# jackroos/VL-BERT

Measured on AMD Instinct MI355X. Metric: samples/sec VL-BERT-base pretrain (seq 64+36 regions) at 1/2/4/8 MI355X, higher is better.
Workload: dtype bf16; 1 GPU; VL-BERT-base 12-layer pretrain step (fwd+bwd+clip+AdamW), 64 text + 36 regions, precomputed 2048-d region features, dropout on; global_batch=256, per_gpu_batch=256, per_gpu_caption_samples=256, per_gpu_text_only_samples=0, module=ResNetVLBERTForPretraining, seq_len=101, parallelism=dp1, hipgraph=False, arch=gfx950:sramecc+:xnack-, cus=256, forced_exchange=False, ranks=1

## Files before the change

### vl-bert_amd/csrc/gemm_p8.hip

```cpp
#include <math.h>
#include <stdlib.h>
#include <string.h>

#include <type_traits>

#include "gemm_params.h"

#ifndef VLB_P8_LN_SB
#define VLB_P8_LN_SB 2
#endif
#ifndef VLB_P8_SIDE_DEPTH
#define VLB_P8_SIDE_DEPTH 1
#endif
#ifndef VLB_P8_WDRAIN
#define VLB_P8_WDRAIN 1
#endif

namespace {

template <int OFF>
__device__ __forceinline__ void p8_lds_read(bf16x8& dst, uint32_t vaddr) {
  asm volatile("ds_read_b128 %0, %1 offset:%2" : "=v"(dst) : "v"(vaddr), "n"(OFF));
}

template <int OFF>
__device__ __forceinline__ void p8_lds_write_f4(uint32_t vaddr, const f32x4& v) {
  asm volatile("ds_write_b128 %0, %1 offset:%2" : : "v"(vaddr), "v"(v), "n"(OFF) : "memory");
}

template <int OFF>
__device__ __forceinline__ void p8_lds_read_f4(f32x4& dst, uint32_t vaddr) {
  asm volatile("ds_read_b128 %0, %1 offset:%2" : "=v"(dst) : "v"(vaddr), "n"(OFF));
}

template <int OFF>
__device__ __forceinline__ void p8_stage_read(f32x4& x0, f32x4& x1, uint32_t a0, uint32_t a1) {
  asm volatile("ds_read_b128 %0, %2 offset:%4\n\tds_read_b128 %1, %3 offset:%4\n\ts_waitcnt lgkmcnt(0)"
               : "=&v"(x0), "=&v"(x1) : "v"(a0), "v"(a1), "n"(OFF) : "memory");
}

template <int I, int N, typename F>
__device__ __forceinline__ void p8_static_for(F&& f) {
  if constexpr (I < N) {
    f(std::integral_constant<int, I>{});
    p8_static_for<I + 1, N>(f);
  }
}

__device__ __forceinline__ void p8_barrier() {
  asm volatile("" ::: "memory");
  __builtin_amdgcn_s_barrier();
  asm volatile("" ::: "memory");
}

template <int EPI>
__device__ __forceinline__ void p8_epilogue8(const GemmParams& p, float (&v)[8], const float (&b8)[8], int m, int n, uint32_t seed,
                                             const uint4& side, const float2 ms = make_float2(0.f, 0.f), const float* g8 = nullptr,
                                             const float* be8 = nullptr) {
#pragma unroll
  for (int e = 0; e < 8; ++e) v[e] += b8[e];
  if (EPI == 1) {
    float d[8];
#pragma unroll
    for (int e = 0; e < 8; e += 2) {
      vlb_f2 g2, d2;
      gelu_both2((vlb_f2){v[e], v[e + 1]}, g2, d2);
      v[e] = g2.x; v[e + 1] = g2.y;
      d[e] = d2.x; d[e + 1] = d2.y;
    }
    if (p.pre) {
      const uint4 dv = make_uint4(pack2bf(d[0], d[1]), pack2bf(d[2], d[3]), pack2bf(d[4], d[5]), pack2bf(d[6], d[7]));
      vlb_store_nt((uint4*)(p.pre + (long)m * p.ldpre + n), dv);
    }
  } else if (EPI == 2) {
    v[0] *= bflo(side.x); v[1] *= bfhi(side.x); v[2] *= bflo(side.y); v[3] *= bfhi(side.y);
    v[4] *= bflo(side.z); v[5] *= bfhi(side.z); v[6] *= bflo(side.w); v[7] *= bfhi(side.w);
  } else if (EPI == 5) {
#pragma unroll
    for (int e = 0; e < 8; ++e) v[e] = fmaxf(v[e], 0.f);
  }
  if (EPI == 3 || EPI == 6) {
    const uint32_t idx = (uint32_t)m * (uint32_t)p.N + (uint32_t)n;
    if ((idx & 1u) == 0) {
#pragma unroll
      for (int q = 0; q < 4; ++q) {
        const uint32_t h = vlb_rng_pair(seed, p.tag, (idx >> 1) + q);
        v[2 * q] = ((h & 0xffffu) >= p.drop_thr) ? v[2 * q] * p.drop_scale : 0.f;
        v[2 * q + 1] = ((h >> 16) >= p.drop_thr) ? v[2 * q + 1] * p.drop_scale : 0.f;
      }
    } else {
#pragma unroll
      for (int e = 0; e < 8; ++e) v[e] = vlb_keep(seed, p.tag, idx + e, p.drop_thr) ? v[e] * p.drop_scale : 0.f;
    }
  }
  if (EPI == 3 || EPI == 4 || EPI == 8) {
    v[0] += bflo(side.x); v[1] += bfhi(side.x); v[2] += bflo(side.y); v[3] += bfhi(side.y);
    v[4] += bflo(side.z); v[5] += bfhi(side.z); v[6] += bflo(side.w); v[7] += bfhi(side.w);
  }
  if (EPI == 8) {
#pragma unroll
    for (int e = 0; e < 8; ++e) v[e] = fmaxf(v[e], 0.f);
  }
  if (EPI == 10) {
    const float a[8] = {bflo(side.x), bfhi(side.x), bflo(side.y), bfhi(side.y), bflo(side.z), bfhi(side.z), bflo(side.w), bfhi(side.w)};
#pragma unroll
    for (int e = 0; e < 8; ++e) v[e] = a[e] > 0.f ? v[e] : 0.f;
  }
  if (EPI == 6 || EPI == 7) {
    const float z[8] = {hlo(side.x), hhi(side.x), hlo(side.y), hhi(side.y), hlo(side.z), hhi(side.z), hlo(side.w), hhi(side.w)};
#pragma unroll
    for (int e = 0; e < 8; ++e) v[e] += fmaf((z[e] - ms.x) * ms.y, g8[e], be8[e]);
  }
}

template <int EPI>
__device__ __forceinline__ float p8_epilogue1(const GemmParams& p, float v, int m, int n, uint32_t seed) {
  if (p.bias) v += p.bias[n];
  if (EPI == 1) {
    float g, d;
    gelu_both(v, g, d);
    if (p.pre) p.pre[(long)m * p.ldpre + n] = f2bf(d);
    v = g;
  } else if (EPI == 2) {
    v *= bf2f(p.aux[(long)m * p.ldaux + n]);
  } else if (EPI == 5) {
    v = fmaxf(v, 0.f);
  }
  if (EPI == 3 || EPI == 6) v = vlb_keep(seed, p.tag, (uint32_t)m * (uint32_t)p.N + (uint32_t)n, p.drop_thr) ? v * p.drop_scale : 0.f;
  if (EPI == 3 || EPI == 4 || EPI == 8) v += bf2f(p.res[(long)m * p.ldres + n]);
  if (EPI == 8) v = fmaxf(v, 0.f);
  if (EPI == 10) v = bf2f(p.aux[(long)m * p.ldaux + n]) > 0.f ? v : 0.f;
  if (EPI == 6 || EPI == 7)
    v += fmaf((h2f(p.res[(long)m * p.ldres + n]) - p.res_stats[2 * (long)m]) * p.res_stats[2 * (long)m + 1], p.res_gamma[n], p.res_beta[n]);
  return v;
}

template <int FMH, int EPI, int KF>
__device__ __forceinline__ void p8_drain(const GemmParams& p, f32x4 (&acc)[2 * FMH][4], uint32_t slab, int m0, int n0, int wm, int wn,
                                         int lane, int tid, uint32_t seed) {
  constexpr int AH = 32 * FMH, NF = 2 * FMH;
  constexpr bool ALT = (KF == 0);
  constexpr bool LNRES = (EPI == 6 || EPI == 7);
  constexpr int FPR = ALT ? 1 : KF;
  constexpr int ROUNDS = ALT ? 2 * NF : (NF + FPR - 1) / FPR;
  constexpr int PASSES = ALT ? 1 : 2 * FPR;
  constexpr bool SIDE = (EPI == 2 || EPI == 3 || EPI == 4 || EPI == 6 || EPI == 7 || EPI == 8 || EPI == 10);
  constexpr bool PRE_NEXT = SIDE && (PASSES <= 2);
  constexpr int SB = PRE_NEXT ? PASSES : (FMH == 5 ? (LNRES ? VLB_P8_LN_SB : 4) : PASSES);
  asm volatile("" : "+v"(tid));
  lane = tid & 63;
  const int frow = lane & 15;
  const int wrow = (ALT ? 0 : wm * 16) + frow;
  uint32_t wr[4];
#pragma unroll
  for (int cj = 0; cj < 4; ++cj) {
#if VLB_P8_WDRAIN
    const int c = wn * 16 + (cj >> 1) * 8 + (cj & 1) * 4 + (lane >> 4);
#else
    const int c = (cj >> 1) * 32 + wn * 8 + (cj & 1) * 4 + (lane >> 4);
#endif
    wr[cj] = slab + (uint32_t)(wrow * 1024 + ((c ^ (frow & 7)) << 4));
  }
  const int q = tid & 31, rho = tid >> 5;
  const uint32_t rd0 = slab + (uint32_t)(rho * 1024 + (((2 * q) ^ (rho & 7)) << 4));
  const uint32_t rd1 = slab + (uint32_t)(rho * 1024 + (((2 * q + 1) ^ (rho & 7)) << 4));
  const int n = n0 + q * 8;
  const bool full8 = n + 8 <= p.N;
  bf16_t* const C = (bf16_t*)p.C;
  float b8[8] = {0.f, 0.f, 0.f, 0.f, 0.f, 0.f, 0.f, 0.f};
  if (p.bias && full8) {
    const float4 b0 = *(const float4*)(p.bias + n), b1 = *(const float4*)(p.bias + n + 4);
    b8[0] = b0.x; b8[1] = b0.y; b8[2] = b0.z; b8[3] = b0.w; b8[4] = b1.x; b8[5] = b1.y; b8[6] = b1.z; b8[7] = b1.w;
  }
  constexpr bool HOIST_GB = LNRES;
  float g8[8], be8[8];
  if constexpr (LNRES) {
#pragma unroll
    for (int e = 0; e < 8; ++e) g8[e] = be8[e] = 0.f;
    if (HOIST_GB && full8) {
      const float4 a0 = *(const float4*)(p.res_gamma + n), a1 = *(const float4*)(p.res_gamma + n + 4);
      const float4 c0 = *(const float4*)(p.res_beta + n), c1 = *(const float4*)(p.res_beta + n + 4);
      g8[0] = a0.x; g8[1] = a0.y; g8[2] = a0.z; g8[3] = a0.w; g8[4] = a1.x; g8[5] = a1.y; g8[6] = a1.z; g8[7] = a1.w;
      be8[0] = c0.x; be8[1] = c0.y; be8[2] = c0.z; be8[3] = c0.w; be8[4] = c1.x; be8[5] = c1.y; be8[6] = c1.z; be8[7] = c1.w;
    }
  }
  const bool f16out = p.c_f16 != 0;
  auto row_of = [&](int r, int pp) {
    const int f = ALT ? 0 : (pp >> 1), g = ALT ? (r & 1) : (pp & 1);
    const int R = ALT ? (r >> 1) : (r * FPR + f);
    const int ha = R / FMH, i = R - ha * FMH;
    return m0 + ha * AH + g * FMH * 16 + i * 16 + rho;
  };
  auto frag_valid = [&](int r, int pp) { return ALT ? true : (r * FPR + (pp >> 1) < NF); };
  auto load_side = [&](int r, int pp) {
    uint4 sd = make_uint4(0, 0, 0, 0);
    if constexpr (SIDE) {
      const int m = row_of(r, pp);
      if (frag_valid(r, pp) && m < p.M && full8) {
        if (EPI == 2 || EPI == 10) sd = vlb_load_nt((const uint4*)(p.aux + (long)m * p.ldaux + n));
        else sd = *(const uint4*)(p.res + (long)m * p.ldres + n);
      }
    }
    return sd;
  };
  auto load_ms = [&](int r, int pp) {
    float2 ms = make_float2(0.f, 0.f);
    if constexpr (LNRES) {
      const int m = min(max(row_of(r, pp), 0), p.M - 1);
      ms = *(const float2*)(p.res_stats + 2 * (long)m);
    }
    return ms;
  };
  uint4 side[2][SB];
  float2 mss[2][SB];
  if constexpr (PRE_NEXT) {
#pragma unroll
    for (int pp = 0; pp < PASSES; ++pp) {
      side[0][pp] = load_side(0, pp);
      mss[0][pp] = load_ms(0, pp);
    }
  }
  p8_static_for<0, ROUNDS>([&](auto r_c) {
    constexpr int r = decltype(r_c)::value;
    if constexpr (SIDE && !PRE_NEXT) {
#pragma unroll
      for (int pp = 0; pp < SB; ++pp) {
        side[0][pp] = load_side(r, pp);
        mss[0][pp] = load_ms(r, pp);
      }
    }
    if (!ALT || wm == (r & 1)) {
      p8_static_for<0, FPR>([&](auto f_c) {
        constexpr int f = decltype(f_c)::value;
        constexpr int R = ALT ? (r >> 1) : (r * FPR + f);
        if constexpr (R < NF) {
          const uint32_t o = (uint32_t)(f * 32 * 1024);
          p8_lds_write_f4<0>(wr[0] + o, acc[R][0]);
          p8_lds_write_f4<0>(wr[1] + o, acc[R][1]);
          p8_lds_write_f4<0>(wr[2] + o, acc[R][2]);
          p8_lds_write_f4<0>(wr[3] + o, acc[R][3]);
        }
      });
    }
    asm volatile("s_waitcnt lgkmcnt(0)" ::: "memory");
    p8_barrier();
    if constexpr (PRE_NEXT) {
      if (r + 1 < ROUNDS) {
#pragma unroll
        for (int pp = 0; pp < PASSES; ++pp) {
          side[(r + 1) & 1][pp] = load_side(r + 1, pp);
          mss[(r + 1) & 1][pp] = load_ms(r + 1, pp);
        }
      }
    }
#pragma unroll
    for (int pp = 0; pp < PASSES; ++pp) {
      if constexpr (SIDE && !PRE_NEXT) {
        if (pp > 0 && pp % SB == 0) {
#pragma unroll
          for (int k = 0; k < SB; ++k) {
            side[0][k] = load_side(r, pp + k);
            mss[0][k] = load_ms(r, pp + k);
          }
        }
      }
      if (!frag_valid(r, pp)) continue;
      const int m = row_of(r, pp);
      f32x4 x0, x1;
      p8_stage_read<0>(x0, x1, rd0 + (uint32_t)(pp * 16 * 1024), rd1 + (uint32_t)(pp * 16 * 1024));
      if (m < p.M && n < p.N) {
        float v[8] = {x0[0], x0[1], x0[2], x0[3], x1[0], x1[1], x1[2], x1[3]};
        if (full8) {
          const uint4 sd = SIDE ? (PRE_NEXT ? side[r & 1][pp] : side[0][pp % SB]) : make_uint4(0, 0, 0, 0);
          if constexpr (LNRES) {
            const float2 ms = PRE_NEXT ? mss[r & 1][pp] : mss[0][pp % SB];
            if constexpr (!HOIST_GB) {
              const float4 a0 = *(const float4*)(p.res_gamma + n), a1 = *(const float4*)(p.res_gamma + n + 4);
              const float4 c0 = *(const float4*)(p.res_beta + n), c1 = *(const float4*)(p.res_beta + n + 4);
              g8[0] = a0.x; g8[1] = a0.y; g8[2] = a0.z; g8[3] = a0.w; g8[4] = a1.x; g8[5] = a1.y; g8[6] = a1.z; g8[7] = a1.w;
              be8[0] = c0.x; be8[1] = c0.y; be8[2] = c0.z; be8[3] = c0.w; be8[4] = c1.x; be8[5] = c1.y; be8[6] = c1.z; be8[7] = c1.w;
            }
            p8_epilogue8<EPI>(p, v, b8, m, n, seed, sd, ms, g8, be8);
          } else {
            p8_epilogue8<EPI>(p, v, b8, m, n, seed, sd);
          }
          const uint4 o4 = make_uint4(pack2o(v[0], v[1], f16out), pack2o(v[2], v[3], f16out), pack2o(v[4], v[5], f16out), pack2o(v[6], v[7], f16out));
          if (p.ablate != 2) *(uint4*)(C + (long)m * p.ldc + n) = o4;
          else if (o4.x == 0x12345678u && o4.y == 0x9abcdef0u) C[0] = 1;
        } else {
          for (int e = 0; e < 8 && n + e < p.N; ++e) {
            const float o = p8_epilogue1<EPI>(p, v[e], m, n + e, seed);
            C[(long)m * p.ldc + n + e] = f16out ? f2h(o) : f2bf(o);
          }
        }
      }
    }
    if (r + 1 < ROUNDS) p8_barrier();
  });
  asm volatile("" ::"v"(b8[0]), "v"(b8[4]));
}

template <int FMH, int EPI, bool EDGE>
__device__ __forceinline__ void p8_drain_w(const GemmParams& p, f32x4 (&acc)[2 * FMH][4], uint32_t slab, int m0, int n0, int wm, int wn,
                                           int tid, uint32_t seed) {
  constexpr int AH = 32 * FMH, NF = 2 * FMH, NU = 2 * NF;
  constexpr bool LNRES = (EPI == 6 || EPI == 7);
  constexpr bool SIDE = (EPI == 2 || EPI == 3 || EPI == 4 || EPI == 6 || EPI == 7 || EPI == 8 || EPI == 10);
  asm volatile("" : "+v"(tid));
  const int lane = tid & 63, frow = lane & 15;
  const uint32_t mine = slab + (uint32_t)((tid >> 6) * 2048);
  uint32_t wr[4];
#pragma unroll
  for (int j = 0; j < 4; ++j) wr[j] = mine + (uint32_t)((frow & 7) * 256 + (((j * 4 + (lane >> 4)) ^ (frow & 7)) << 4));
  const bool upper = (frow >> 3) != 0;
  const int rr = lane >> 3, cq = lane & 7;
  const uint32_t rd0 = mine + (uint32_t)(rr * 256 + (((2 * cq) ^ rr) << 4));
  const uint32_t rd1 = mine + (uint32_t)(rr * 256 + (((2 * cq + 1) ^ rr) << 4));
  const bool f16out = p.c_f16 != 0;
  const int n = n0 + wn * 64 + cq * 8;
  const bool full8 = EDGE ? (n + 8 <= p.N) : true;
  const int mw = m0 + wm * FMH * 16 + rr;
  auto uoff = [](int u) { return ((u >> 1) / FMH) * AH + ((u >> 1) % FMH) * 16 + (u & 1) * 8; };
  bf16_t* const Cl = (bf16_t*)p.C + (long)mw * p.ldc + n;
  const bf16_t* const Sl = !SIDE ? nullptr : ((EPI == 2 || EPI == 10) ? p.aux + (long)mw * p.ldaux + n : p.res + (long)mw * p.ldres + n);
  const long lds_ = (EPI == 2 || EPI == 10) ? p.ldaux : p.ldres;
  const float* const Ml = LNRES ? p.res_stats + 2 * (long)mw : nullptr;
  float b8[8] = {0.f, 0.f, 0.f, 0.f, 0.f, 0.f, 0.f, 0.f}, g8[8], be8[8];
  auto consts = [&]() {
    if (p.bias && full8) {
      const float4 b0 = *(const float4*)(p.bias + n), b1 = *(const float4*)(p.bias + n + 4);
      b8[0] = b0.x; b8[1] = b0.y; b8[2] = b0.z; b8[3] = b0.w; b8[4] = b1.x; b8[5] = b1.y; b8[6] = b1.z; b8[7] = b1.w;
    }
    if constexpr (LNRES) {
#pragma unroll
      for (int e = 0; e < 8; ++e) g8[e] = be8[e] = 0.f;
      if (full8) {
        const float4 a0 = *(const float4*)(p.res_gamma + n), a1 = *(const float4*)(p.res_gamma + n + 4);
        const float4 c0 = *(const float4*)(p.res_beta + n), c1 = *(const float4*)(p.res_beta + n + 4);
        g8[0] = a0.x; g8[1] = a0.y; g8[2] = a0.z; g8[3] = a0.w; g8[4] = a1.x; g8[5] = a1.y; g8[6] = a1.z; g8[7] = a1.w;
        be8[0] = c0.x; be8[1] = c0.y; be8[2] = c0.z; be8[3] = c0.w; be8[4] = c1.x; be8[5] = c1.y; be8[6] = c1.z; be8[7] = c1.w;
      }
    }
  };
  auto load_side = [&](int u, uint4& sd, float2& ms) {
    if constexpr (SIDE) {
      if (!EDGE || (mw + uoff(u) < p.M && full8)) {
        const uint4* src = (const uint4*)(Sl + uoff(u) * lds_);
        if (EPI == 2 || EPI == 10) sd = vlb_load_nt(src);
        else sd = *src;
        if constexpr (LNRES) ms = *(const float2*)(Ml + 2 * uoff(u));
      }
    }
  };
  auto put = [&](auto u_c) {
    constexpr int u = decltype(u_c)::value, R = u >> 1, hf = u & 1;
    if (upper == (hf != 0)) {
      p8_lds_write_f4<0>(wr[0], acc[R][0]);
      p8_lds_write_f4<0>(wr[1], acc[R][1]);
      p8_lds_write_f4<0>(wr[2], acc[R][2]);
      p8_lds_write_f4<0>(wr[3], acc[R][3]);
    }
  };
  auto finish = [&](int u, const f32x4& x0, const f32x4& x1, const uint4& sd, const float2& ms) {
    const int m = mw + uoff(u);
    if (!EDGE || (m < p.M && n < p.N)) {
      float v[8] = {x0[0], x0[1], x0[2], x0[3], x1[0], x1[1], x1[2], x1[3]};
      if (full8) {
        if constexpr (LNRES) p8_epilogue8<EPI>(p, v, b8, m, n, seed, sd, ms, g8, be8);
        else p8_epilogue8<EPI>(p, v, b8, m, n, seed, sd);
        uint4 o4;
        if (f16out) {
          asm volatile("" ::: "memory");
          o4 = make_uint4(pack2h(v[0], v[1]), pack2h(v[2], v[3]), pack2h(v[4], v[5]), pack2h(v[6], v[7]));
        } else {
          o4 = make_uint4(pack2bf(v[0], v[1]), pack2bf(v[2], v[3]), pack2bf(v[4], v[5]), pack2bf(v[6], v[7]));
        }
        *(uint4*)(Cl + (p.ablate != 2 ? uoff(u) * (long)p.ldc : 0L)) = o4;
      } else {
        for (int e = 0; e < 8 && n + e < p.N; ++e) {
          const float o = p8_epilogue1<EPI>(p, v[e], m, n + e, seed);
          Cl[uoff(u) * (long)p.ldc + e] = f16out ? f2h(o) : f2bf(o);
        }
      }
    }
  };
  constexpr int DEPTH = (EPI == 2 || EPI == 10) ? VLB_P8_SIDE_DEPTH : 1, RING = DEPTH + 1;
  uint4 side[RING];
  float2 mst[RING];
#pragma unroll
  for (int d = 0; d < RING; ++d) {
    side[d] = make_uint4(0, 0, 0, 0);
    mst[d] = make_float2(0.f, 0.f);
  }
  consts();
  p8_static_for<0, (DEPTH < NU ? DEPTH : NU)>([&](auto d_c) {
    constexpr int d = decltype(d_c)::value;
    load_side(d, side[d % RING], mst[d % RING]);
  });
  put(std::integral_constant<int, 0>{});
  p8_static_for<0, NU>([&](auto u_c) {
    constexpr int u = decltype(u_c)::value;
    f32x4 x0, x1;
    p8_stage_read<0>(x0, x1, rd0, rd1);
    if constexpr (u + DEPTH < NU) load_side(u + DEPTH, side[(u + DEPTH) % RING], mst[(u + DEPTH) % RING]);
    if constexpr (u + 1 < NU) put(std::integral_constant<int, u + 1>{});
    finish(u, x0, x1, side[u % RING], mst[u % RING]);
  });
  asm volatile("" ::"v"(b8[0]), "v"(b8[4]));
}

template <int FMH, int EPI, bool KEEPB>
__global__ __launch_bounds__(512, 2) void gemm_nt_p8_kernel(const GemmParams p) {
  constexpr int AH = 32 * FMH;
  constexpr int BM = 2 * AH, BN = 256;
  constexpr int AHB = AH * 128, BHB = 128 * 128;
  constexpr int OFF_A0 = 0, OFF_A1 = AHB, OFF_B0 = 2 * AHB, OFF_B1 = 2 * AHB + BHB;
  constexpr int BUF = 2 * AHB + 2 * BHB;
  constexpr int STG = 2 * BUF;
  constexpr int SR = (163840 - STG) / 1024 >= 32 ? 32 : (163840 - STG) / 1024;
  constexpr int NLA = (AH * 8 + 511) / 512;
  constexpr int VM_AHEAD = (AH * 8) / 512 + 2;
  static_assert(SR == 32 || SR == 16, "staging slab");
  extern __shared__ __attribute__((aligned(16))) char smem[];

  const int tid = threadIdx.x, lane = tid & 63;
  const int wave = __builtin_amdgcn_readfirstlane(tid >> 6);
  const int wm = wave >> 2, wn = wave & 3;
  const int nt = p.ntm * p.ntn;
  const int nk = p.K >> 6;
  if ((int)blockIdx.x >= nt) return;
  unsigned long long* const stamps = (unsigned long long*)(EPI == 1 ? (void*)p.aux : (void*)p.pre);
  const bool stamp = (p.ablate == 4) && stamps;
  unsigned long long t_main = 0, t_epi = 0, t_mark = 0;
  if (stamp && tid == 0) {
    unsigned long long* t = stamps + 8 * blockIdx.x;
    t[0] = __builtin_readcyclecounter();
    t[1] = __builtin_amdgcn_s_memrealtime();
  }

  auto tile_of = [&](int w, int& m0, int& n0) {
    int tile_m, tile_n;
    vlb_tile_of(vlb_xcd_order(w, nt), p.ntm, p.ntn, p.tile_group, tile_m, tile_n);
    m0 = tile_m * BM;
    n0 = tile_n * BN;
  };

  const __amdgpu_buffer_rsrc_t rsA = __builtin_amdgcn_make_buffer_rsrc((void*)p.A, 0, 0x7FFFFFFF, 0x00020000);
  const __amdgpu_buffer_rsrc_t rsB = __builtin_amdgcn_make_buffer_rsrc((void*)p.B, 0, 0x7FFFFFFF, 0x00020000);
  const int ldaB = (int)p.lda * 2, ldbB = (int)p.ldb * 2;
  const int kcb = (((tid & 7) ^ ((tid >> 4) & 7)) << 4);
  const int rowA = (tid >> 3) * ldaB + kcb, maxA = (p.M - 1) * ldaB + kcb;
#if VLB_P8_WDRAIN
  const int rowB = ((tid >> 8) * 64 + ((tid >> 3) & 31)) * ldbB + kcb, maxB = (p.N - 1) * ldbB + kcb;
#else
  const int rowB = (tid >> 3) * ldbB + kcb, maxB = (p.N - 1) * ldbB + kcb;
#endif
  int w_p = blockIdx.x, kt_p = 0, pm0 = 0, pn0 = 0;
  auto setup = [&](int w) { tile_of(w, pm0, pn0); };
  auto stage = [&](auto which_c, auto buf_c) {
    constexpr int WHICH = decltype(which_c)::value, B_ = decltype(buf_c)::value;
    const int koff = kt_p * 128;
    if constexpr (WHICH < 2) {
      char* dst = smem + B_ * BUF + (WHICH == 0 ? OFF_A0 : OFF_A1);
#pragma unroll
      for (int it = 0; it < NLA; ++it) {
        if (it * 512 + 511 < AH * 8 || wave < (AH * 8 - it * 512) / 64) {
          const int vo = min((pm0 + WHICH * AH + it * 64) * ldaB + rowA, maxA);
          __builtin_amdgcn_raw_ptr_buffer_load_lds(rsA, LDS_PTR(dst + (it * 512 + wave * 64) * 16), 16, vo, koff, 0, 0);
        }
      }
    } else {
      char* dst = smem + B_ * BUF + (WHICH == 2 ? OFF_B0 : OFF_B1);
#pragma unroll
      for (int it = 0; it < 2; ++it) {
#if VLB_P8_WDRAIN
        const int vo = min((pn0 + (WHICH - 2) * 32 + it * 128) * ldbB + rowB, maxB);
#else
        const int vo = min((pn0 + (WHICH - 2) * 128 + it * 64) * ldbB + rowB, maxB);
#endif
        __builtin_amdgcn_raw_ptr_buffer_load_lds(rsB, LDS_PTR(dst + (it * 512 + wave * 64) * 16), 16, vo, koff, 0, 0);
      }
    }
  };
  auto advance = [&]() {
    if (++kt_p == nk) {
      if (w_p + (int)gridDim.x < nt) {
        kt_p = 0;
        w_p += gridDim.x;
        setup(w_p);
      } else {
        kt_p = nk - 1;
      }
    }
  };
  constexpr int ORD1 = KEEPB ? 2 : 3, ORD2 = KEEPB ? 3 : 1, ORD3 = KEEPB ? 1 : 2;
  using I0 = std::integral_constant<int, 0>;
  using I1 = std::integral_constant<int, 1>;
  using W0 = std::integral_constant<int, 0>;
  using W1 = std::integral_constant<int, ORD1>;
  using W2 = std::integral_constant<int, ORD2>;
  using W3 = std::integral_constant<int, ORD3>;

  f32x4 acc[2 * FMH][4];
  bf16x8 af[FMH][2], bfr[2][2], bkeep[2][2];
  const int frow = lane & 15;
  const uint32_t c0 = (uint32_t)((((lane >> 4) ^ (frow >> 1)) << 4));
  const uint32_t lds0 = (uint32_t)(uintptr_t)LDS_PTR(smem);
  const uint32_t a_rd = lds0 + (uint32_t)((wm * FMH * 16 + frow) * 128) + c0;
  const uint32_t b_rd = lds0 + (uint32_t)(OFF_B0 + (wn * 32 + frow) * 128) + c0;

  auto read_a = [&](auto buf_c, auto half_c) {
    constexpr int B_ = decltype(buf_c)::value, H_ = decltype(half_c)::value;
    const uint32_t v0 = a_rd + B_ * BUF, v1 = v0 ^ 64u;
    constexpr int O = H_ * AHB;
    p8_lds_read<O + 0 * 2048>(af[0][0], v0); p8_lds_read<O + 0 * 2048>(af[0][1], v1);
    p8_lds_read<O + 1 * 2048>(af[1][0], v0); p8_lds_read<O + 1 * 2048>(af[1][1], v1);
    p8_lds_read<O + 2 * 2048>(af[2][0], v0); p8_lds_read<O + 2 * 2048>(af[2][1], v1);
    if constexpr (FMH >= 4) {
      p8_lds_read<O + 3 * 2048>(af[3][0], v0); p8_lds_read<O + 3 * 2048>(af[3][1], v1);
    }
    if constexpr (FMH == 5) {
      p8_lds_read<O + 4 * 2048>(af[4][0], v0); p8_lds_read<O + 4 * 2048>(af[4][1], v1);
    }
  };
  auto read_b = [&](auto buf_c, auto half_c, bf16x8 (&dst)[2][2]) {
    constexpr int B_ = decltype(buf_c)::value, H_ = decltype(half_c)::value;
    const uint32_t v0 = b_rd + B_ * BUF, v1 = v0 ^ 64u;
    constexpr int O = H_ * BHB;
    p8_lds_read<O>(dst[0][0], v0); p8_lds_read<O>(dst[0][1], v1);
    p8_lds_read<O + 2048>(dst[1][0], v0); p8_lds_read<O + 2048>(dst[1][1], v1);
  };
  auto compute = [&](auto ha_c, auto hb_c, bf16x8 (&bq)[2][2]) {
    constexpr int HA = decltype(ha_c)::value, HB = decltype(hb_c)::value;
    if constexpr (FMH == 3) {
      asm volatile("s_waitcnt lgkmcnt(0)"
                   : "+v"(af[0][0]), "+v"(af[0][1]), "+v"(af[1][0]), "+v"(af[1][1]), "+v"(af[2][0]), "+v"(af[2][1]), "+v"(bq[0][0]),
                     "+v"(bq[0][1]), "+v"(bq[1][0]), "+v"(bq[1][1]));
    } else if constexpr (FMH == 4) {
      asm volatile("s_waitcnt lgkmcnt(0)"
                   : "+v"(af[0][0]), "+v"(af[0][1]), "+v"(af[1][0]), "+v"(af[1][1]), "+v"(af[2][0]), "+v"(af[2][1]), "+v"(af[3][0]),
                     "+v"(af[3][1]), "+v"(bq[0][0]), "+v"(bq[0][1]), "+v"(bq[1][0]), "+v"(bq[1][1]));
    } else {
      asm volatile("s_waitcnt lgkmcnt(0)"
                   : "+v"(af[0][0]), "+v"(af[0][1]), "+v"(af[1][0]), "+v"(af[1][1]), "+v"(af[2][0]), "+v"(af[2][1]), "+v"(af[3][0]),
                     "+v"(af[3][1]), "+v"(af[4][0]), "+v"(af[4][1]), "+v"(bq[0][0]), "+v"(bq[0][1]), "+v"(bq[1][0]), "+v"(bq[1][1]));
    }
    __builtin_amdgcn_sched_barrier(0);
    __builtin_amdgcn_s_setprio(1);
#pragma unroll
    for (int ks = 0; ks < 2; ++ks)
#pragma unroll
      for (int i = 0; i < FMH; ++i)
#pragma unroll
        for (int j = 0; j < 2; ++j)
          acc[HA * FMH + i][HB * 2 + j] = VLB_MFMA_16x16x32(bq[j][ks], af[i][ks], acc[HA * FMH + i][HB * 2 + j], 0, 0, 0);
    __builtin_amdgcn_s_setprio(0);
    __builtin_amdgcn_sched_barrier(0);
  };

  setup(w_p);
  stage(W0{}, I0{}); stage(W1{}, I0{}); stage(W2{}, I0{}); stage(W3{}, I0{});
  advance();
  stage(W0{}, I1{}); stage(W1{}, I1{});
  __builtin_amdgcn_s_waitcnt(0x0F70 | VM_AHEAD);
  p8_barrier();
  if (wm == 1) p8_barrier();

  int g = 0;
  const uint32_t seed = (EPI == 3 || EPI == 6) ? *p.seed : 0u;
  for (int w = blockIdx.x; w < nt; w += gridDim.x) {
#pragma unroll
    for (int i = 0; i < 2 * FMH; ++i)
#pragma unroll
      for (int j = 0; j < 4; ++j) acc[i][j] = (f32x4){0.f, 0.f, 0.f, 0.f};

    if (stamp) t_mark = __builtin_readcyclecounter();
    for (int kt = 0; kt < nk; kt += 2, g += 2) {
      if constexpr (KEEPB) read_b(I0{}, I0{}, bkeep); else read_b(I0{}, I0{}, bfr);
      __builtin_amdgcn_sched_barrier(0);
      read_a(I0{}, I0{});
      stage(W2{}, I1{});
      p8_barrier();
      if constexpr (KEEPB) compute(I0{}, I0{}, bkeep); else compute(I0{}, I0{}, bfr);
      p8_barrier();
      read_b(I0{}, I1{}, bfr);
      stage(W3{}, I1{});
      p8_barrier();
      compute(I0{}, I1{}, bfr);
      p8_barrier();
      read_a(I0{}, I1{});
      advance();
      stage(W0{}, I0{});
      p8_barrier();
      compute(I1{}, I1{}, bfr);
      p8_barrier();
      if constexpr (!KEEPB) read_b(I0{}, I0{}, bfr);
      stage(W1{}, I0{});
      __builtin_amdgcn_s_waitcnt(0x0F70 | VM_AHEAD);
      p8_barrier();
      if constexpr (KEEPB) compute(I1{}, I0{}, bkeep); else compute(I1{}, I0{}, bfr);
      p8_barrier();
      if constexpr (KEEPB) read_b(I1{}, I0{}, bkeep); else read_b(I1{}, I0{}, bfr);
      __builtin_amdgcn_sched_barrier(0);
      read_a(I1{}, I0{});
      stage(W2{}, I0{});
      p8_barrier();
      if constexpr (KEEPB) compute(I0{}, I0{}, bkeep); else compute(I0{}, I0{}, bfr);
      p8_barrier();
      read_b(I1{}, I1{}, bfr);
      stage(W3{}, I0{});
      p8_barrier();
      compute(I0{}, I1{}, bfr);
      p8_barrier();
      read_a(I1{}, I1{});
      advance();
      stage(W0{}, I1{});
      p8_barrier();
      compute(I1{}, I1{}, bfr);
      p8_barrier();
      if constexpr (!KEEPB) read_b(I1{}, I0{}, bfr);
      stage(W1{}, I1{});
      __builtin_amdgcn_s_waitcnt(0x0F70 | VM_AHEAD);
      p8_barrier();
      if constexpr (KEEPB) compute(I1{}, I0{}, bkeep); else compute(I1{}, I0{}, bfr);
      p8_barrier();
    }
    if (wm == 0) p8_barrier();
    if (stamp) {
      const unsigned long long now = __builtin_readcyclecounter();
      t_main += now - t_mark;
      t_mark = now;
    }

    int m0, n0;
    tile_of(w, m0, n0);
    if (p.ablate == 1) {
#if VLB_P8_WDRAIN
    } else if ((w + (int)gridDim.x < nt || EPI == 0 || (p.p8_flags & 2)) && !(FMH == 5 && (EPI == 6 || EPI == 7))) {
      if (m0 + BM <= p.M && n0 + BN <= p.N) p8_drain_w<FMH, EPI, false>(p, acc, lds0 + STG, m0, n0, wm, wn, tid, seed);
      else p8_drain_w<FMH, EPI, true>(p, acc, lds0 + STG, m0, n0, wm, wn, tid, seed);
#endif
    } else if (w + (int)gridDim.x >= nt) {
      __builtin_amdgcn_s_waitcnt(0x0F70);
      p8_barrier();
      p8_drain<FMH, EPI, (STG >= 131072 ? 4 : 3)>(p, acc, lds0, m0, n0, wm, wn, lane, tid, seed);
    } else {
      p8_drain<FMH, EPI, (SR == 32 ? 1 : 0)>(p, acc, lds0 + STG, m0, n0, wm, wn, lane, tid, seed);
    }
    if (p.p8_flags & 1) __builtin_amdgcn_s_waitcnt(0x0F70);
    p8_barrier();
    if (wm == 1 && w + (int)gridDim.x < nt) p8_barrier();
    if (stamp) t_epi += __builtin_readcyclecounter() - t_mark;
  }
  __builtin_amdgcn_s_waitcnt(0x0F70);
  if (stamp && tid == 0) {
    unsigned long long* t = stamps + 8 * blockIdx.x;
    t[2] = __builtin_readcyclecounter();
    t[3] = __builtin_amdgcn_s_memrealtime();
    t[4] = t_main;
    t[5] = t_epi;
    t[6] = (unsigned long long)((nt - (int)blockIdx.x + (int)gridDim.x - 1) / (int)gridDim.x);
  }
}

template <int FMH, bool KEEPB>
int p8_launch_epi(GemmParams& p, int epi, hipStream_t stream) {
  const int wgs = vlb_opt(VLB_OPT_P8_WGS);
  const int rc = dispatch_epi(epi, std::integer_sequence<int, 0, 1, 2, 3, 4, 5, 6, 7, 8, 10>{}, VLB_ERR_ARG, [&](auto e) {
    return launch_persistent<gemm_nt_p8_kernel<FMH, decltype(e)::value, KEEPB>>(163840, 512, 64 * FMH, 256, (wgs >= 8 && wgs <= 256) ? (wgs & ~7) : 256,
                                                                                vlb_opt(VLB_OPT_P8_GROUP), p, 1, stream, "vlb_gemm_nt_bf16(p8)", true);
  });
  return rc < 0 ? rc : 1;
}

inline bool aligned16(const void* q) { return ((uintptr_t)q & 15) == 0; }

}

int vlb_gemm_p8_try(GemmParams& p, hipStream_t stream) {
  const int mode = vlb_opt(VLB_OPT_P8_MODE), min_tiles = vlb_opt(VLB_OPT_P8_MIN_TILES);
  if (!mode || p.out_f32 != 0 || p.c_split_stride != 0) return 0;
  if ((p.K % 128) != 0 || p.k_per_split < p.K) return 0;
  int epi;
  if (p.act == 0 && p.res && p.res_stats) epi = p.drop_thr ? 6 : 7;
  else if (p.act == 0) epi = p.res ? (p.drop_thr ? 3 : 4) : (p.drop_thr ? -1 : 0);
  else if (p.act == 4) epi = 1;
  else if (p.act == 5) epi = 2;
  else if (p.act == 2) epi = 5;
  else if (p.act == 7 && p.res && !p.drop_thr) epi = 8;
  else if (p.act == 8 && !p.res && !p.drop_thr) epi = 10;
  else epi = -1;
  if (epi < 0) return 0;
  if ((p.ldc % 8) || !aligned16(p.C) || (p.lda % 8) || (p.ldb % 8) || !aligned16(p.A) || !aligned16(p.B)) return 0;
  if (p.res && ((p.ldres % 8) || !aligned16(p.res))) return 0;
  if ((epi == 2 || epi == 10) && ((p.ldaux % 8) || !aligned16(p.aux))) return 0;
  if (epi == 1 && p.pre && ((p.ldpre % 8) || !aligned16(p.pre))) return 0;
  if (p.bias && ((uintptr_t)p.bias & 15)) return 0;
  if (p.res_stats && (((uintptr_t)p.res_gamma & 15) || ((uintptr_t)p.res_beta & 15) || ((uintptr_t)p.res_stats & 7))) return 0;
  if ((long)p.M * p.lda * 2 >= (1L << 31) || (long)p.N * p.ldb * 2 >= (1L << 31)) return 0;
  const long nn = vlb_cdiv(p.N, 256);
  const long t3 = (long)vlb_cdiv(p.M, 192) * nn, t4 = (long)vlb_cdiv(p.M, 256) * nn, t5 = (long)vlb_cdiv(p.M, 320) * nn;
  const double c3 = (double)((t3 + 255) / 256) * 192.0 * 1.15, c4 = (double)((t4 + 255) / 256) * 256.0, c5 = (double)((t5 + 255) / 256) * 320.0;
  const bool ok3 = t3 >= min_tiles, ok4 = t4 >= min_tiles || (t4 >= 128 && p.K >= 1536), ok5 = t5 >= min_tiles;
  int fmh = 0;
  double best = 1e30;
  if (ok4) { fmh = 4; best = c4; }
  if (ok5 && c5 < 0.97 * best) { fmh = 5; best = c5; }
  if (ok3 && vlb_opt(VLB_OPT_P8_TILE192) && c3 < 0.97 * best) { fmh = 3; best = c3; }
  if (mode == 3 || mode == 4 || mode == 5) fmh = mode;
  if (!fmh) return 0;
  p.ablate = vlb_opt(VLB_OPT_P8_ABLATE);
  p.p8_flags = (vlb_opt(VLB_OPT_P8_DRAIN) & 1) | (vlb_opt(VLB_OPT_P8_LASTW) ? 2 : 0);
  if (fmh == 3) return p8_launch_epi<3, true>(p, epi, stream);
  if (fmh == 5) return p8_launch_epi<5, false>(p, epi, stream);
  return vlb_opt(VLB_OPT_P8_KEEPB) ? p8_launch_epi<4, true>(p, epi, stream) : p8_launch_epi<4, false>(p, epi, stream);
}
```

### vl-bert_amd/csrc/options.h

```cpp
#pragma once

#define VLB_OPTIONS(X)                                                                                                                  \
                                                                                 \
                                \
  X(P8_MODE, "p8_mode", "VLB_GEMM_P8", 1)                                                                                               \
                         \
  X(P8_KEEPB, "p8_keepb", "VLB_GEMM_P8_KEEPB", 1)                                                                                       \
                                                                                             \
  X(P8_GROUP, "p8_group", "VLB_GEMM_P8_GROUP", 2)                                                                                       \
                       \
  X(P8_MIN_TILES, "p8_min_tiles", "VLB_GEMM_P8_MIN_TILES", 160)                                                                         \
              \
  X(P8_WGS, "p8_wgs", "VLB_GEMM_P8_WGS", 256)                                                                                           \
                                         \
  X(P8_ABLATE, "p8_ablate", nullptr, 0)                                                                                                 \
                                                                                       \
  X(P8_TILE192, "p8_tile192", "VLB_GEMM_P8_192", 1)                                                                                     \
                                                    \
  X(P8_DRAIN, "p8_drain", "VLB_GEMM_P8_DRAIN", 0)                                                                                       \
                                         \
  X(P8_LASTW, "p8_lastw", "VLB_GEMM_P8_LASTW", 0)                                                                                       \
                                                                                                    \
                                                                   \
  X(NT_RING, "nt_ring", "VLB_GEMM_NT_RING", 1)                                                                                          \
                                                         \
  X(NT_STAGGER, "nt_stagger", "VLB_GEMM_NT_STAGGER", 0)                                                                                 \
                                                     \
  X(TILE_GROUP, "tile_group", "VLB_GEMM_TILE_GROUP", 4)                                                                                 \
                 \
  X(RESIDENT, "resident", "VLB_GEMM_RESIDENT", 512)                                                                                     \
               \
  X(EPI_SPECIALISE, "epi_specialise", "VLB_GEMM_EPI_SPECIALISE", 1)                                                                     \
   \
  X(NT_256, "nt_256", "VLB_GEMM_256", 1)                                                                                                \
                                                                                      \
  X(NT_256_GROUP, "nt_256_group", "VLB_GEMM_256_GROUP", 2)                                                                              \
                                                                           \
                                                                \
  X(TN_GROUP, "tn_group", "VLB_GEMM_TN_GROUP", -1)                                                                                      \
                                                                                     \
  X(TN_WAVES8, "tn_waves8", "VLB_GEMM_TN_WAVES8", 1)                                                                                    \
                                                                           \
                                                                                                     \
  X(TN8_MODE, "tn8_mode", "VLB_GEMM_TN8", 1)                                                                                            \
                                                                  \
  X(TN8_WGS, "tn8_wgs", "VLB_GEMM_TN8_WGS", 256)                                                                                        \
                                                                                           \
  X(TN8_UNEVEN, "tn8_uneven", "VLB_GEMM_TN8_UNEVEN", 0)                                                                                 \
                                                                                                   \
  X(TN8_M32, "tn8_m32", "VLB_GEMM_TN8_M32", 0)                                                                                          \
                                                         \
  X(TN8_ABLATE, "tn8_ablate", nullptr, 0)                                                                                               \
                                                                \
  X(TN8_GROUP, "tn8_group", "VLB_GEMM_TN8_GROUP", 0)                                                                                    \
                                                    \
                        \
  X(LN_FWD_ROWS, "ln_fwd_rows", "VLB_LN_FWD_ROWS", 0)                                                                                   \
                                  \
  X(LN_BWD4, "ln_bwd4", "VLB_LN_BWD4", 1)                                                                                               \
                                            \
  X(ATTN_BWD2, "attn_bwd2", "VLB_ATTN_BWD2", 1)

enum VlbOpt {
#define VLB_OPT_ID(id, name, env, dflt) VLB_OPT_##id,
  VLB_OPTIONS(VLB_OPT_ID)
#undef VLB_OPT_ID
  VLB_OPT_COUNT
};

int vlb_opt(VlbOpt o);
bool vlb_opt_set(const char* name, int value);
```

Baseline: 13900 samples/s.

## Add interior-tile GEMM drain with deep side-tensor prefetch ring and no bounds checks

For full interior tiles in the last-wave slab drain, dispatches to a specialised drain that skips the M/N bounds checks. For aux/residual epilogues it also streams the side-tensor rows through a deeper prefetch ring, with explicit vmcnt waits, so global loads overlap the LDS staging and epilogue math. Dropout epilogues take the paired-RNG path unconditionally on this interior path. This adds code size and register pressure from the ring, and can be turned off with a new option that forces the edge path.

Result: no change. 13900 samples/s (-0.0%).

```diff
diff --git a/vl-bert_amd/csrc/gemm_p8.hip b/vl-bert_amd/csrc/gemm_p8.hip
--- a/vl-bert_amd/csrc/gemm_p8.hip
+++ b/vl-bert_amd/csrc/gemm_p8.hip
@@ -53,7 +53,7 @@
   asm volatile("" ::: "memory");
 }
 
-template <int EPI>
+template <int EPI, bool PAIRS = false>
 __device__ __forceinline__ void p8_epilogue8(const GemmParams& p, float (&v)[8], const float (&b8)[8], int m, int n, uint32_t seed,
                                              const uint4& side, const float2 ms = make_float2(0.f, 0.f), const float* g8 = nullptr,
                                              const float* be8 = nullptr) {
@@ -81,7 +81,7 @@
   }
   if (EPI == 3 || EPI == 6) {
     const uint32_t idx = (uint32_t)m * (uint32_t)p.N + (uint32_t)n;
-    if ((idx & 1u) == 0) {
+    if (PAIRS || (idx & 1u) == 0) {
 #pragma unroll
       for (int q = 0; q < 4; ++q) {
         const uint32_t h = vlb_rng_pair(seed, p.tag, (idx >> 1) + q);
@@ -135,22 +135,23 @@
   return v;
 }
 
+#ifndef VLB_P8_SLAB_LEAD
+#define VLB_P8_SLAB_LEAD 8
+#endif
+
 template <int FMH, int EPI, int KF>
-__device__ __forceinline__ void p8_drain(const GemmParams& p, f32x4 (&acc)[2 * FMH][4], uint32_t slab, int m0, int n0, int wm, int wn,
-                                         int lane, int tid, uint32_t seed) {
-  constexpr int AH = 32 * FMH, NF = 2 * FMH;
-  constexpr bool ALT = (KF == 0);
-  constexpr bool LNRES = (EPI == 6 || EPI == 7);
-  constexpr int FPR = ALT ? 1 : KF;
-  constexpr int ROUNDS = ALT ? 2 * NF : (NF + FPR - 1) / FPR;
-  constexpr int PASSES = ALT ? 1 : 2 * FPR;
-  constexpr bool SIDE = (EPI == 2 || EPI == 3 || EPI == 4 || EPI == 6 || EPI == 7 || EPI == 8 || EPI == 10);
-  constexpr bool PRE_NEXT = SIDE && (PASSES <= 2);
-  constexpr int SB = PRE_NEXT ? PASSES : (FMH == 5 ? (LNRES ? VLB_P8_LN_SB : 4) : PASSES);
+__device__ __forceinline__ void p8_drain_inside(const GemmParams& p, f32x4 (&acc)[2 * FMH][4], uint32_t slab, int m0, int n0, int wm, int wn,
+                                                int tid, uint32_t seed) {
+  constexpr int NF = 2 * FMH, ROUNDS = (NF + KF - 1) / KF, PASSES = 2 * KF, TOTAL = 2 * NF;
+  constexpr bool LNRES = (EPI == 6 || EPI == 7), AUX = (EPI == 2 || EPI == 10);
+  static_assert(KF >= 3 && (AUX || LNRES || EPI == 3 || EPI == 4 || EPI == 8), "side-tensor epilogues through the slab over the idle ring");
+  constexpr int LEAD = VLB_P8_SLAB_LEAD, RING = LEAD + 1;
+  constexpr int LEAD0 = FMH == 5 ? (LNRES ? VLB_P8_LN_SB : 4) : (LNRES ? 4 : 2 * KF);
+  constexpr int LPR = LNRES ? 2 : 1;
+  static_assert(LEAD >= 1 && LEAD0 <= RING && LEAD0 >= 1, "ring");
   asm volatile("" : "+v"(tid));
-  lane = tid & 63;
-  const int frow = lane & 15;
-  const int wrow = (ALT ? 0 : wm * 16) + frow;
+  const int lane = tid & 63, frow = lane & 15;
+  const int wrow = wm * 16 + frow;
   uint32_t wr[4];
 #pragma unroll
   for (int cj = 0; cj < 4; ++cj) {
@@ -164,8 +165,120 @@
   const int q = tid & 31, rho = tid >> 5;
   const uint32_t rd0 = slab + (uint32_t)(rho * 1024 + (((2 * q) ^ (rho & 7)) << 4));
   const uint32_t rd1 = slab + (uint32_t)(rho * 1024 + (((2 * q + 1) ^ (rho & 7)) << 4));
+  const int n = n0 + q * 8, mt = m0 + rho;
+  bf16_t* const Cl = (bf16_t*)p.C + (long)mt * p.ldc + n;
+  const bf16_t* const Sl = AUX ? p.aux + (long)mt * p.ldaux + n : p.res + (long)mt * p.ldres + n;
+  const long lds_ = AUX ? p.ldaux : p.ldres;
+  const float* const Ml = LNRES ? p.res_stats + 2 * (long)mt : nullptr;
+  const bool f16out = p.c_f16 != 0;
+  float b8[8] = {0.f, 0.f, 0.f, 0.f, 0.f, 0.f, 0.f, 0.f}, g8[8], be8[8];
+  if (p.bias) {
+    const float4 b0 = *(const float4*)(p.bias + n), b1 = *(const float4*)(p.bias + n + 4);
+    b8[0] = b0.x; b8[1] = b0.y; b8[2] = b0.z; b8[3] = b0.w; b8[4] = b1.x; b8[5] = b1.y; b8[6] = b1.z; b8[7] = b1.w;
+  }
+  if constexpr (LNRES) {
+    const float4 a0 = *(const float4*)(p.res_gamma + n), a1 = *(const float4*)(p.res_gamma + n + 4);
+    const float4 c0 = *(const float4*)(p.res_beta + n), c1 = *(const float4*)(p.res_beta + n + 4);
+    g8[0] = a0.x; g8[1] = a0.y; g8[2] = a0.z; g8[3] = a0.w; g8[4] = a1.x; g8[5] = a1.y; g8[6] = a1.z; g8[7] = a1.w;
+    be8[0] = c0.x; be8[1] = c0.y; be8[2] = c0.z; be8[3] = c0.w; be8[4] = c1.x; be8[5] = c1.y; be8[6] = c1.z; be8[7] = c1.w;
+  }
+  auto toff = [](int g) constexpr {
+    const int r = g / PASSES, pp = g % PASSES, R = r * KF + (pp >> 1), ha = R / FMH;
+    return ha * 32 * FMH + (pp & 1) * FMH * 16 + (R - ha * FMH) * 16;
+  };
+  auto load_row = [&](int off) {
+    const uint4* src = (const uint4*)(Sl + off * lds_);
+    return AUX ? vlb_load_nt(src) : *src;
+  };
+  uint4 side[RING], tail;
+  float2 mss[RING];
+  auto request = [&](auto g_c) {
+    constexpr int g = decltype(g_c)::value, off = toff(g);
+    side[g % RING] = load_row(off);
+    if constexpr (LNRES) mss[g % RING] = *(const float2*)(Ml + 2 * off);
+  };
+  asm volatile("; p8_drain_inside begin" ::: "memory");
+  p8_static_for<0, LEAD0>([&](auto g_c) { request(g_c); });
+  p8_static_for<0, ROUNDS>([&](auto r_c) {
+    constexpr int r = decltype(r_c)::value;
+    p8_static_for<0, KF>([&](auto f_c) {
+      constexpr int f = decltype(f_c)::value, R = r * KF + f;
+      if constexpr (R < NF) {
+        const uint32_t o = (uint32_t)(f * 32 * 1024);
+        p8_lds_write_f4<0>(wr[0] + o, acc[R][0]);
+        p8_lds_write_f4<0>(wr[1] + o, acc[R][1]);
+        p8_lds_write_f4<0>(wr[2] + o, acc[R][2]);
+        p8_lds_write_f4<0>(wr[3] + o, acc[R][3]);
+      }
+    });
+    asm volatile("s_waitcnt lgkmcnt(0)" ::: "memory");
+    p8_barrier();
+    p8_static_for<r * PASSES, (r * PASSES + PASSES < TOTAL ? r * PASSES + PASSES : TOTAL)>([&](auto g_c) {
+      constexpr int g = decltype(g_c)::value, off = toff(g);
+      constexpr int had = g == 0 ? LEAD0 : (g + LEAD < TOTAL ? g + LEAD : TOTAL), have = g + 1 + LEAD < TOTAL ? g + 1 + LEAD : TOTAL;
+      p8_static_for<had, have>([&](auto n_c) { request(n_c); });
+      if constexpr (have - g - 1 > 0) {
+        asm volatile("s_waitcnt vmcnt(%0)" ::"n"((have - g - 1) * LPR) : "memory");
+      } else {
+        tail = load_row(off);
+        asm volatile("s_waitcnt vmcnt(1)" ::: "memory");
+      }
+      __builtin_amdgcn_sched_barrier(0);
+      f32x4 x0, x1;
+      p8_stage_read<0>(x0, x1, rd0 + (uint32_t)((g % PASSES) * 16 * 1024), rd1 + (uint32_t)((g % PASSES) * 16 * 1024));
+      float v[8] = {x0[0], x0[1], x0[2], x0[3], x1[0], x1[1], x1[2], x1[3]};
+      if constexpr (LNRES) p8_epilogue8<EPI>(p, v, b8, mt + off, n, seed, side[g % RING], mss[g % RING], g8, be8);
+      else p8_epilogue8<EPI>(p, v, b8, mt + off, n, seed, side[g % RING]);
+      uint4 o4;
+      if (f16out) {
+        asm volatile("" ::: "memory");
+        o4 = make_uint4(pack2h(v[0], v[1]), pack2h(v[2], v[3]), pack2h(v[4], v[5]), pack2h(v[6], v[7]));
+      } else {
+        o4 = make_uint4(pack2bf(v[0], v[1]), pack2bf(v[2], v[3]), pack2bf(v[4], v[5]), pack2bf(v[6], v[7]));
+      }
+      *(uint4*)(Cl + (p.ablate != 2 ? off * (long)p.ldc : 0L)) = o4;
+    });
+    if constexpr (r + 1 < ROUNDS) p8_barrier();
+  });
+  asm volatile("; p8_drain_inside end" ::"v"(tail.x), "v"(b8[0]), "v"(b8[4]) : "memory");
+}
+
+template <int FMH, int EPI, int KF, bool EDGE = true>
+__device__ __forceinline__ void p8_drain(const GemmParams& p, f32x4 (&acc)[2 * FMH][4], uint32_t slab, int m0, int n0, int wm, int wn,
+                                         int lane, int tid, uint32_t seed) {
+  constexpr bool LNRES = (EPI == 6 || EPI == 7);
+  if constexpr (!EDGE && !(LNRES || EPI == 3)) {
+    p8_drain_inside<FMH, EPI, KF>(p, acc, slab, m0, n0, wm, wn, tid, seed);
+    return;
+  }
+  static_assert(EDGE || KF >= 3, "the interior form belongs to the slab over the idle ring");
+  constexpr int AH = 32 * FMH, NF = 2 * FMH;
+  constexpr bool ALT = (KF == 0);
+  constexpr int FPR = ALT ? 1 : KF;
+  constexpr int ROUNDS = ALT ? 2 * NF : (NF + FPR - 1) / FPR;
+  constexpr int PASSES = ALT ? 1 : 2 * FPR;
+  constexpr bool SIDE = (EPI == 2 || EPI == 3 || EPI == 4 || EPI == 6 || EPI == 7 || EPI == 8 || EPI == 10);
+  constexpr bool PRE_NEXT = SIDE && (PASSES <= 2);
+  constexpr int SB = PRE_NEXT ? PASSES : (FMH == 5 ? (LNRES ? VLB_P8_LN_SB : 4) : ((!EDGE && LNRES && FMH == 4) ? 4 : PASSES));
+  asm volatile("" : "+v"(tid));
+  lane = tid & 63;
+  const int frow = lane & 15;
+  const int wrow = (ALT ? 0 : wm * 16) + frow;
+  uint32_t wr[4];
+#pragma unroll
+  for (int cj = 0; cj < 4; ++cj) {
+#if VLB_P8_WDRAIN
+    const int c = wn * 16 + (cj >> 1) * 8 + (cj & 1) * 4 + (lane >> 4);
+#else
+    const int c = (cj >> 1) * 32 + wn * 8 + (cj & 1) * 4 + (lane >> 4);
+#endif
+    wr[cj] = slab + (uint32_t)(wrow * 1024 + ((c ^ (frow & 7)) << 4));
+  }
+  const int q = tid & 31, rho = tid >> 5;
+  const uint32_t rd0 = slab + (uint32_t)(rho * 1024 + (((2 * q) ^ (rho & 7)) << 4));
+  const uint32_t rd1 = slab + (uint32_t)(rho * 1024 + (((2 * q + 1) ^ (rho & 7)) << 4));
   const int n = n0 + q * 8;
-  const bool full8 = n + 8 <= p.N;
+  const bool full8 = !EDGE || n + 8 <= p.N;
   bf16_t* const C = (bf16_t*)p.C;
   float b8[8] = {0.f, 0.f, 0.f, 0.f, 0.f, 0.f, 0.f, 0.f};
   if (p.bias && full8) {
@@ -196,7 +309,7 @@
     uint4 sd = make_uint4(0, 0, 0, 0);
     if constexpr (SIDE) {
       const int m = row_of(r, pp);
-      if (frag_valid(r, pp) && m < p.M && full8) {
+      if (frag_valid(r, pp) && (!EDGE || (m < p.M && full8))) {
         if (EPI == 2 || EPI == 10) sd = vlb_load_nt((const uint4*)(p.aux + (long)m * p.ldaux + n));
         else sd = *(const uint4*)(p.res + (long)m * p.ldres + n);
       }
@@ -213,6 +326,7 @@
   };
   uint4 side[2][SB];
   float2 mss[2][SB];
+  if constexpr (!EDGE) asm volatile("; p8_drain_inside begin" ::: "memory");
   if constexpr (PRE_NEXT) {
 #pragma unroll
     for (int pp = 0; pp < PASSES; ++pp) {
@@ -266,9 +380,10 @@
       }
       if (!frag_valid(r, pp)) continue;
       const int m = row_of(r, pp);
+      if constexpr (!EDGE) __builtin_amdgcn_sched_barrier(0);
       f32x4 x0, x1;
       p8_stage_read<0>(x0, x1, rd0 + (uint32_t)(pp * 16 * 1024), rd1 + (uint32_t)(pp * 16 * 1024));
-      if (m < p.M && n < p.N) {
+      if (!EDGE || (m < p.M && n < p.N)) {
         float v[8] = {x0[0], x0[1], x0[2], x0[3], x1[0], x1[1], x1[2], x1[3]};
         if (full8) {
           const uint4 sd = SIDE ? (PRE_NEXT ? side[r & 1][pp] : side[0][pp % SB]) : make_uint4(0, 0, 0, 0);
@@ -280,14 +395,15 @@
               g8[0] = a0.x; g8[1] = a0.y; g8[2] = a0.z; g8[3] = a0.w; g8[4] = a1.x; g8[5] = a1.y; g8[6] = a1.z; g8[7] = a1.w;
               be8[0] = c0.x; be8[1] = c0.y; be8[2] = c0.z; be8[3] = c0.w; be8[4] = c1.x; be8[5] = c1.y; be8[6] = c1.z; be8[7] = c1.w;
             }
-            p8_epilogue8<EPI>(p, v, b8, m, n, seed, sd, ms, g8, be8);
+            p8_epilogue8<EPI, !EDGE>(p, v, b8, m, n, seed, sd, ms, g8, be8);
           } else {
-            p8_epilogue8<EPI>(p, v, b8, m, n, seed, sd);
+            p8_epilogue8<EPI, !EDGE>(p, v, b8, m, n, seed, sd);
           }
           const uint4 o4 = make_uint4(pack2o(v[0], v[1], f16out), pack2o(v[2], v[3], f16out), pack2o(v[4], v[5], f16out), pack2o(v[6], v[7], f16out));
-          if (p.ablate != 2) *(uint4*)(C + (long)m * p.ldc + n) = o4;
+          if constexpr (!EDGE) *(uint4*)(C + (long)(p.ablate != 2 ? m : m0 + rho) * p.ldc + n) = o4;
+          else if (p.ablate != 2) *(uint4*)(C + (long)m * p.ldc + n) = o4;
           else if (o4.x == 0x12345678u && o4.y == 0x9abcdef0u) C[0] = 1;
-        } else {
+        } else if constexpr (EDGE) {
           for (int e = 0; e < 8 && n + e < p.N; ++e) {
             const float o = p8_epilogue1<EPI>(p, v[e], m, n + e, seed);
             C[(long)m * p.ldc + n + e] = f16out ? f2h(o) : f2bf(o);
@@ -297,6 +413,7 @@
     }
     if (r + 1 < ROUNDS) p8_barrier();
   });
+  if constexpr (!EDGE) asm volatile("; p8_drain_inside end" ::: "memory");
   asm volatile("" ::"v"(b8[0]), "v"(b8[4]));
 }
 
@@ -643,7 +760,17 @@
     } else if (w + (int)gridDim.x >= nt) {
       __builtin_amdgcn_s_waitcnt(0x0F70);
       p8_barrier();
-      p8_drain<FMH, EPI, (STG >= 131072 ? 4 : 3)>(p, acc, lds0, m0, n0, wm, wn, lane, tid, seed);
+      constexpr int KFL = STG >= 131072 ? 4 : 3;
+      constexpr bool EDGE_W = FMH == 4 && EPI == 7 && VLB_P8_WDRAIN;
+      constexpr bool SIDE = (EPI == 2 || EPI == 3 || EPI == 4 || EPI == 6 || EPI == 7 || EPI == 8 || EPI == 10) && !(FMH == 4 && EPI == 7 && !EDGE_W);
+      const bool inside = SIDE && m0 + BM <= p.M && n0 + BN <= p.N && !(p.p8_flags & 4) && !((EPI == 3 || EPI == 6) && (p.N & 1));
+      if constexpr (SIDE) {
+        if (inside) p8_drain<FMH, EPI, KFL, false>(p, acc, lds0, m0, n0, wm, wn, lane, tid, seed);
+      }
+      if (!inside) {
+        if constexpr (EDGE_W) p8_drain_w<FMH, EPI, true>(p, acc, lds0 + STG, m0, n0, wm, wn, tid, seed);
+        else p8_drain<FMH, EPI, KFL, true>(p, acc, lds0, m0, n0, wm, wn, lane, tid, seed);
+      }
     } else {
       p8_drain<FMH, EPI, (SR == 32 ? 1 : 0)>(p, acc, lds0 + STG, m0, n0, wm, wn, lane, tid, seed);
     }
@@ -710,7 +837,7 @@
   if (mode == 3 || mode == 4 || mode == 5) fmh = mode;
   if (!fmh) return 0;
   p.ablate = vlb_opt(VLB_OPT_P8_ABLATE);
-  p.p8_flags = (vlb_opt(VLB_OPT_P8_DRAIN) & 1) | (vlb_opt(VLB_OPT_P8_LASTW) ? 2 : 0);
+  p.p8_flags = (vlb_opt(VLB_OPT_P8_DRAIN) & 1) | (vlb_opt(VLB_OPT_P8_LASTW) ? 2 : 0) | (vlb_opt(VLB_OPT_P8_SLAB_EDGE) ? 4 : 0);
   if (fmh == 3) return p8_launch_epi<3, true>(p, epi, stream);
   if (fmh == 5) return p8_launch_epi<5, false>(p, epi, stream);
   return vlb_opt(VLB_OPT_P8_KEEPB) ? p8_launch_epi<4, true>(p, epi, stream) : p8_launch_epi<4, false>(p, epi, stream);
diff --git a/vl-bert_amd/csrc/options.h b/vl-bert_amd/csrc/options.h
--- a/vl-bert_amd/csrc/options.h
+++ b/vl-bert_amd/csrc/options.h
@@ -20,6 +20,8 @@
   X(P8_DRAIN, "p8_drain", "VLB_GEMM_P8_DRAIN", 0)                                                                                       \
                                          \
   X(P8_LASTW, "p8_lastw", "VLB_GEMM_P8_LASTW", 0)                                                                                       \
+    \
+  X(P8_SLAB_EDGE, "p8_slab_edge", "VLB_GEMM_P8_SLAB_EDGE", 0)                                                                           \
                                                                                                     \
                                                                    \
   X(NT_RING, "nt_ring", "VLB_GEMM_NT_RING", 1)                                                                                          \
```
